# wenz116/lang2seg

Hardware: AMD Instinct MI355X
Metric: train images/sec (cycle loss on), 600×1000 input, at 1/2/4/8 MI355X (higher is better)
Workload: dtype bf16; 1 GPU; train_cycle.sh step: ResNet-101 C4 + 7 spatial dynamic filters + att2in2 cycle loss, 600x1000 image, 20-token expression (V=3349), 12000->2000 proposals, 256 RoIs, per-GPU batch 1; variant=cycle, parallelism=dp1

## Files before the change

### include/lang2seg_hip.h

```cpp
#ifndef LANG2SEG_HIP_H
#define LANG2SEG_HIP_H
#include <stdint.h>
#ifdef __HIPCC__
#include <hip/hip_runtime.h>
#else
typedef struct ihipStream_t* hipStream_t;
#endif
#ifdef __cplusplus
extern "C" {
#endif

#define L2S_F32 0
#define L2S_BF16 1

int l2s_version(void);

#define L2S_CONV_RELU 1
#define L2S_CONV_OUT_F32 4
#define L2S_CONV_DECONV2X2 8
#define L2S_CONV_SCATTER 16
#define L2S_ALGO_AUTO 0
#define L2S_ALGO_STAGED 1
#define L2S_ALGO_DMA 2
#define L2S_ALGO_DMA_STAMPED 4
// ... 274 lines not shown
int l2s_prep_geometry(int h, int w, int target_size, int max_size, double* scale, int* oh, int* ow);
int l2s_prep_image(const uint8_t* img_bgr, int h, int w, double mean_b, double mean_g, double mean_r, double scale,
                   int oh, int ow, float* out, hipStream_t s);
long l2s_rle_ws_words(int total_counts, int oh, int ow);
int l2s_rle_to_mask(const uint32_t* cnts, const int* offs, int n, int total_counts, int h, int w, int oh, int ow,
                    uint32_t* ws, uint8_t* out, hipStream_t s);

typedef struct { int roi; int cls; float box[4]; int hit; int reserved; long long I; long long U; } l2s_eval_record;
int l2s_eval_pick(const float* cls_prob, const float* bbox_pred, const float* rois, const int* nkeep, int post, int ncls, float im_scale,
                  int im_h, int im_w, const float* gt_box, int bbox_reg, l2s_eval_record* rec, float* mask_roi, int* mask_label, hipStream_t s);
int l2s_eval_mask_iou(const float* mask_prob, int ms, l2s_eval_record* rec, const uint8_t* gt, int Hs, int Ws, int ih, int iw,
                      uint8_t* canvas, hipStream_t s);

int l2s_stream_fork(hipStream_t from, hipStream_t to);
int l2s_event_record(int slot, hipStream_t s);
int l2s_event_wait(int slot, hipStream_t s);
int l2s_memset_async(void* p, int value, size_t bytes, hipStream_t s);
int l2s_memcpy_d2d_async(void* dst, const void* src, size_t bytes, hipStream_t s);
void* l2s_tape_begin(const hipStream_t* streams, int n);
int l2s_tape_end(void* tape);
long l2s_tape_size(void* tape);
int l2s_tape_run(void* tape, const hipStream_t* streams, int n);
int l2s_tape_pause(int on);
int l2s_tape_mark(void);
int l2s_tape_time_event(hipStream_t s);
int l2s_time_event_elapsed(int a, int b, float* ms);
int l2s_tape_segments(void* tape);
int l2s_tape_run_segment(void* tape, const hipStream_t* streams, int n, int seg);
int l2s_tape_destroy(void* tape);

typedef struct { long offset; long count; int row_len; int weight_decay; long rowscale_off; float lr_mult;
                 int chunk0;
                 int flags;
                 int reserved; } l2s_sgd_seg;
int l2s_sgd_momentum_range(float* param, float* grad, float* mom, const l2s_sgd_seg* segs, int nseg, const float* rowscale,
                           float lr, float momentum, float wd, float grad_scale, void* shadow, int shadow_dtype, int flags,
                           long lo, long hi, int chunk_lo, int chunk_hi, hipStream_t s);
int l2s_sgd_momentum_range_g16(float* param, const void* grad_bf16, long grad_lo, float* mom, const l2s_sgd_seg* segs, int nseg, const float* rowscale,
                               float lr, float momentum, float wd, float grad_scale, void* shadow, int shadow_dtype,
                               long lo, long hi, int chunk_lo, int chunk_hi, hipStream_t s);
int l2s_sgd_chunk(void);
int l2s_sgd_momentum(float* param, float* grad, float* mom, const l2s_sgd_seg* segs, int nseg, const float* rowscale,
                     float lr, float momentum, float wd, float grad_scale, void* shadow ,
                     int shadow_dtype, int clear_grad ,
                     hipStream_t s);

#ifdef __cplusplus
}
#endif
#endif
```

### lang2seg_amd/_lib.py

```python
import ctypes as C
import os

_HERE = os.path.dirname(os.path.abspath(__file__))
LIB_PATH = os.path.join(_HERE, 'lib', 'liblang2seg_hip.so')
F32, BF16 = 0, 1

vp, i32, i64, f32, u64, sz = C.c_void_p, C.c_int, C.c_long, C.c_float, C.c_uint64, C.c_size_t


class ConvDesc(C.Structure):
    _fields_ = [('x', vp), ('w', vp), ('y', vp), ('bias', vp), ('add', vp), ('ref', vp),
                ('n_img', i32), ('IH', i32), ('IW', i32), ('Cin', i32), ('OH', i32), ('OW', i32), ('Cout', i32),
                ('KH', i32), ('KW', i32), ('stride', i32), ('pad', i32),
                ('ldx', i32), ('ldy', i32), ('ldadd', i32), ('ldref', i32), ('flags', i32),
                ('out_h', i32), ('out_w', i32), ('out_stride', i32), ('tile', i32), ('split_k', i32), ('xcd_mode', i32), ('algo', i32), ('ws', vp), ('ws_floats', sz), ('prio', i32)]


class RoiBlock0Desc(C.Structure):
    _fields_ = [('feat', vp), ('rois', vp), ('w1', vp), ('b1', vp), ('w2', vp), ('b2', vp), ('pooled', vp), ('y1', vp), ('y2', vp),
                ('H', i32), ('W', i32), ('C', i32), ('R', i32), ('P', i32), ('N1', i32), ('N2', i32), ('spatial_scale', C.c_float), ('debug', i32)]


class WgradDesc(C.Structure):
    _fields_ = [('dy', vp), ('x', vp), ('dw', vp),
# ... 7 lines not shown
                ('lddy', i32 * 2), ('ldx', i32 * 2), ('dw', vp),
                ('nseg', i32), ('Cin', i32), ('Cout', i32), ('KH', i32), ('KW', i32), ('stride', i32), ('pad', i32),
                ('split', i32), ('ws_off', i64), ('flags', i32), ('reserved', i32)]


class TransposeDesc(C.Structure):
    _fields_ = [('src', vp), ('scale', vp), ('dst', vp), ('Cout', i32), ('taps', i32), ('Cin', i32), ('force_f32', i32)]


class LstmFwdDir(C.Structure):
    _fields_ = [(n, C.c_void_p) for n in ('w_hh', 'b_hh', 'gates_in', 'h_prev', 'c_prev', 'c', 'h', 'act', 'gates_out')]


class LstmBwdDir(C.Structure):
    _fields_ = [(n, C.c_void_p) for n in ('w_hh_T', 'dgates_next', 'dh_ext', 'dc_in', 'act', 'c_prev', 'c', 'dgates', 'dc_prev')]


class Bottleneck64Desc(C.Structure):
    _fields_ = [(n, vp) for n in ('a', 'x', 'w2', 'w3', 'wd', 'w1n', 'b2', 'b3', 'bd', 'b1n', 'y', 'a_next')] + [(n, i32) for n in ('H', 'W', 'Cx')]


class CapRecurFwdArgs(C.Structure):
    _fields_ = [(n, vp) for n in ('w_h2h', 'b_h2h', 'w_h2att', 'b_h2att', 'patt', 'aw', 'ab', 'P', 'b_a2c', 'sums', 'hs', 'cs', 'save', 'tanh_ws', 'wgt', 'state')] + \
               [(n, i32) for n in ('S', 'R', 'AH', 'L')]


class CapRecurBwdArgs(C.Structure):
    _fields_ = [(n, vp) for n in ('w_h2h', 'w_h2att', 'P', 'aw', 'save', 'cs', 'wgt', 'tanh_ws', 'dho', 'dsums', 'da2c', 'ddot', 'datt_h', 'state')] + \
               [(n, i32) for n in ('S', 'R', 'AH', 'L', 'ld_ddot', 'ld_datt_h')]


class SgdSeg(C.Structure):
    _fields_ = [('offset', i64), ('count', i64), ('row_len', i32), ('weight_decay', i32), ('rowscale_off', i64),
                ('lr_mult', f32), ('chunk0', i32), ('flags', i32), ('reserved', i32)]


CONV_RELU, CONV_OUT_F32, CONV_DECONV2X2, CONV_SCATTER = 1, 4, 8, 16
LOSS_RPN_CLS, LOSS_RPN_BOX, LOSS_CLS, LOSS_BOX, LOSS_MASK, LOSS_CAP, LOSS_TOTAL, LOSS_RESPONSE = range(8)

SIGS = {
    'l2s_version': (i32, []),
    'l2s_conv_plan_name': (C.c_char_p, [vp, i32]),
    'l2s_roialign_block0_fwd': (i32, [C.POINTER(RoiBlock0Desc), vp]),
    'l2s_conv_igemm': (i32, [C.POINTER(ConvDesc), i32, vp]),
    'l2s_conv_wgrad': (i32, [C.POINTER(WgradDesc), i32, vp]),
    'l2s_wgrad_ws_bytes': (sz, [C.POINTER(WgradDesc), i32]),
    'l2s_wgrad_variant': (i32, [i32, i32, i32, i32, i32, i32, i32, i64, i32]),
    'l2s_wgrad_tiles': (i64, [i32, i32, i32, i32, i32]),
    'l2s_conv_wgrad_grouped': (i32, [vp, vp, i32, i32, i32, vp, sz, vp]),
    'l2s_weight_cast': (i32, [vp, vp, vp, i32, i32, i32, i32, vp]),
    'l2s_weight_transpose': (i32, [vp, vp, vp, i32, i32, i32, i32, vp]),
    'l2s_colsum': (i32, [vp, i32, i32, i32, vp, vp, i64, i32, vp]),
    'l2s_weight_transpose_batched': (i32, [vp, i32, i32, i32, vp]),
    'l2s_stem_conv': (i32, [vp, vp, vp, vp, vp, i32, i32, i32, i32, i32, vp]),
    'l2s_stem_pack_bytes': (C.c_size_t, []),
    'l2s_stem_pack': (i32, [vp, vp, vp]),
    'l2s_stem_pool_bf16': (i32, [vp, vp, vp, vp, vp, i32, i32, i32, i32, i32, i32, vp]),
    'l2s_maxpool3x3s2': (i32, [vp, vp, i32, i32, i32, i32, i32, i32, vp]),
    'l2s_fill_f32': (i32, [vp, f32, i64, vp]),
    'l2s_cast': (i32, [vp, i32, vp, i32, i64, vp]),
    'l2s_add3': (i32, [vp, vp, vp, vp, i64, i32, vp]),
    'l2s_avgpool_fwd': (i32, [vp, vp, i32, i32, i32, i32, vp]),
    'l2s_avgpool_bwd': (i32, [vp, vp, vp, vp, i32, i32, i32, i32, vp]),
    'l2s_adaptive_pool_fwd': (i32, [vp, vp, vp, i32, i32, i32, i32, i32, i32, i32, vp]),
    'l2s_adaptive_pool_bwd': (i32, [vp, i32, i32, i32, vp, vp, vp, i32, i32, i32, i32, i32, i32, vp]),
    'l2s_mask_downsample': (i32, [vp, vp, i32, i32, i32, i32, vp]),
    'l2s_dropout_mask': (i32, [vp, i64, f32, vp, u64, vp]),
# ... 150 lines not shown
```

### lang2seg_amd/csrc/misc_kernels.hip

```cpp
#include "common.h"
#include "../../include/lang2seg_hip.h"

namespace {

__device__ __forceinline__ uint64_t mix64(uint64_t z) {
  z += 0x9E3779B97F4A7C15ull;
  z = (z ^ (z >> 30)) * 0xBF58476D1CE4E5B9ull;
  z = (z ^ (z >> 27)) * 0x94D049BB133111EBull;
  return z ^ (z >> 31);
}

inline int grid_for(long n, int block = 256, int cap = 2048) {
  long g = (n + block - 1) / block;
  if (g < 1) g = 1;
  return (int)(g > cap ? cap : g);
}

__global__ void weight_cast_kernel(const float* __restrict__ src, const float* __restrict__ scale, void* dst,
                                   long per_row, long total, int dt) {
  for (long i = blockIdx.x * (long)blockDim.x + threadIdx.x; i < total; i += (long)gridDim.x * blockDim.x) {
    float v = src[i];
    if (scale) v *= scale[i / per_row];
    stx(dst, i, dt, v);
  }
// ... 465 lines not shown
  const int bw = x1 - x0, n = (y1 - y0) * bw;
  float s = 0.f;
  for (int i = lane; i < n; i += 64) { int yy = y0 + i / bw, xx = x0 + i % bw; s += (float)mask[(long)yy * W + xx]; }
  s = wave_sum(s);
  if (lane == 0) out[o] = (s / (float)n >= 0.5f) ? 1.f : 0.f;
}

__global__ void counter_inc_kernel(uint64_t* c) { *c += 1; }
__global__ void stamp_kernel(uint64_t* out) { *out = wall_clock64(); }
__global__ void dropout_kernel(float* m, long n, float p, const uint64_t* seed_dev, uint64_t salt) {
  const uint64_t seed = mix64(*seed_dev * 0x9E3779B97F4A7C15ull + salt);
  const float keep = 1.f - p, inv = keep > 0.f ? 1.f / keep : 0.f;
  for (long i = blockIdx.x * (long)blockDim.x + threadIdx.x; i < n; i += (long)gridDim.x * blockDim.x) {
    uint32_t r = (uint32_t)(mix64(seed * 0x100000001B3ull + (uint64_t)i) >> 40);
    m[i] = ((float)r * (1.f / 16777216.f) < keep) ? inv : 0.f;
  }
}
__global__ void keys_kernel(uint32_t* k, long n, const uint64_t* seed_dev, uint64_t salt) {
  const uint64_t seed = mix64(*seed_dev * 0x9E3779B97F4A7C15ull + salt);
  for (long i = blockIdx.x * (long)blockDim.x + threadIdx.x; i < n; i += (long)gridDim.x * blockDim.x)
    k[i] = (uint32_t)(mix64(seed * 0x100000001B3ull + (uint64_t)i) >> 32);
}

constexpr int SGD_CHUNK = 4096;
__device__ __forceinline__ void sgd_elem(float g, float& w, float& m, float rs, float gscale, float lwd, float momentum, float llr) {
  const float gg = g * gscale * rs + lwd * w;
  m = momentum * m + gg;
  w = w - llr * m;
}
__global__ __launch_bounds__(256) void sgd_kernel(float* __restrict__ param, float* __restrict__ grad, float* __restrict__ mom,
                                                  const l2s_sgd_seg* __restrict__ segs, int nseg, const float* __restrict__ rowscale,
                                                  float lr, float momentum, float wd, float gscale, void* shadow, int sdt, int flags,
                                                  long lo, long hi, int chunk_lo, int chunk_hi, const bf16_t* __restrict__ g16, long g16_lo) {
  const bool clear = flags & 1, shadow_only = flags & 2;
  const int c0 = segs[0].chunk0;
  int total = segs[nseg - 1].chunk0 - c0 + (int)((segs[nseg - 1].count + SGD_CHUNK - 1) / SGD_CHUNK);
  if (chunk_hi >= 0 && chunk_hi < total) total = chunk_hi;
  for (int c = (chunk_lo > 0 ? chunk_lo : 0) + blockIdx.x; c < total; c += gridDim.x) {
    int slo = 0, shi = nseg - 1;
    while (slo < shi) {
      const int mid = (slo + shi + 1) >> 1;
      if (segs[mid].chunk0 - c0 <= c) slo = mid; else shi = mid - 1;
    }
    const l2s_sgd_seg sg = segs[slo];
    const long base = (long)(c - (sg.chunk0 - c0)) * SGD_CHUNK;
    const int n = (int)((sg.count - base) < SGD_CHUNK ? (sg.count - base) : SGD_CHUNK);
    const float lwd = sg.weight_decay ? wd : 0.f;
    const float llr = lr * sg.lr_mult;
    const bool clr = clear && !(sg.flags & 1);
    const long o0 = sg.offset + base;
    const bool inside = o0 >= lo && o0 + n <= hi;
    const bool vec = inside && ((sg.offset & 3) == 0) && (sg.rowscale_off < 0 || (sg.row_len & 3) == 0);
    const int nv = vec ? (n >> 2) : 0;
    float4 g4[4], w4[4], m4[4];
#pragma unroll
    for (int j = 0; j < 4; ++j) {
      const int v = threadIdx.x + j * 256;
      if (v < nv) {
        w4[j] = *(const float4*)(param + o0 + 4 * v);
        if (!shadow_only) {
          if (g16) {
            const uint2 pk = *(const uint2*)(g16 + (o0 + 4 * v - g16_lo));
            g4[j] = make_float4(bf2f((bf16_t)(pk.x & 0xffffu)), bf2f((bf16_t)(pk.x >> 16)), bf2f((bf16_t)(pk.y & 0xffffu)), bf2f((bf16_t)(pk.y >> 16)));
          } else g4[j] = *(const float4*)(grad + o0 + 4 * v);
          m4[j] = *(const float4*)(mom + o0 + 4 * v);
        }
      }
    }
#pragma unroll
    for (int j = 0; j < 4; ++j) {
      const int v = threadIdx.x + j * 256;
      if (v >= nv) continue;
      const long o = o0 + 4 * v;
      const float rs = sg.rowscale_off >= 0 ? rowscale[sg.rowscale_off + (unsigned)(base + 4 * v) / (unsigned)sg.row_len] : 1.f;
      float ww[4] = {w4[j].x, w4[j].y, w4[j].z, w4[j].w};
      if (!shadow_only) {
        float gg[4] = {g4[j].x, g4[j].y, g4[j].z, g4[j].w}, mm[4] = {m4[j].x, m4[j].y, m4[j].z, m4[j].w};
#pragma unroll
        for (int e = 0; e < 4; ++e) sgd_elem(gg[e], ww[e], mm[e], rs, gscale, lwd, momentum, llr);
        *(float4*)(mom + o) = make_float4(mm[0], mm[1], mm[2], mm[3]);
        *(float4*)(param + o) = make_float4(ww[0], ww[1], ww[2], ww[3]);
        if (clr && !g16) *(float4*)(grad + o) = make_float4(0.f, 0.f, 0.f, 0.f);
// ... 220 lines not shown
```

### lang2seg_amd/nets/network.py

```python
import numpy as np
import os
import torch

from .. import ops as O
from .._lib import F32, BF16, LOSS_CAP
from ..model.config import cfg
from .params import ParamStore
from . import anchors as ANC


class ConvOp(object):

    def __init__(self, net, wkey, Cin, Cout, k=1, stride=1, pad=0, bias_key=None, need_dgrad=True, group=None, Cout_pad=None, full_map=False):
        self.net, self.wkey, self.Cin, self.Cout, self.k, self.stride, self.pad = net, wkey, Cin, Cout, k, stride, pad
        self.full_map = bool(full_map and k > 1 and pad == 0 and stride == 1)
        self.t_taps, self.t_cin = (1, k * k * Cin) if self.full_map else (k * k, Cin)
        self.bias_key, self.need_dgrad, self.group = bias_key, need_dgrad, group
        self.Np = Cout if Cout_pad is None else Cout_pad
        self.prio = 1 if str(wkey).startswith(('resnet.layer1.', 'resnet.layer2.', 'resnet.layer3.')) and getattr(net, 'chain_prio', True) else 0
        P = net.P
        taps = k * k
        cnt = self.Np * taps * Cin
        if group is not None:
            self.trainable = True
# ... 500 lines not shown
        raise NotImplementedError

    def train(self, mode=True):
        self.training = mode
        return self

    def eval(self):
        return self.train(False)

    def cuda(self):
        return self

    def state_dict(self):
        self.join_update()
        dp = getattr(self, 'dp', None)
        if dp is not None and getattr(dp, 'master_stale', False):
            raise RuntimeError('state_dict() of a sharded data-parallel run: call net.dp.gather_master() on every rank first')
        return self.P.state_dict()

    def load_state_dict(self, sd, strict=False):
        self.join_update()
        self.P.load_state_dict(sd, strict)
        self.refresh_weights(full=True)

    def named_parameters(self):
        from .params import from_internal
        self.join_update()
        dp = getattr(self, 'dp', None)
        if dp is not None and getattr(dp, 'master_stale', False):
            raise RuntimeError('named_parameters() of a sharded data-parallel run: call net.dp.gather_master() on every rank first')
        for k in self.P.trainable:
            yield k, from_internal(k, self.P.view(k), self.P.shapes[k])

    def refresh_weights(self, full=False):
        if full:
            for c in self.convs:
                if not c.trainable:
                    O.weight_cast(c.w_master, c.scale, c.wf, c.Np, c.k * c.k, c.Cin)
        if getattr(self, '_tr_table', None) is None:
            from .._lib import TransposeDesc
            items = [c for c in self.convs if c.wb is not None] + list(getattr(self, 'extra_transposes', []))
            arr = (TransposeDesc * len(items))()
            for i, c in enumerate(items):
                arr[i].src, arr[i].scale, arr[i].dst = c.w_master.data_ptr(), (c.scale.data_ptr() if c.scale is not None else None), c.wb.data_ptr()
                arr[i].Cout, arr[i].taps, arr[i].Cin, arr[i].force_f32 = c.Np, getattr(c, 't_taps', c.k * c.k), getattr(c, 't_cin', c.Cin), int(getattr(c, 'force_f32', 0))
                if self.dt == BF16 and isinstance(c, ConvOp) and c.trainable and not arr[i].force_f32:
                    arr[i].src, arr[i].scale, arr[i].force_f32 = c.wf.data_ptr(), None, 2
            self._tr_table = torch.frombuffer(bytearray(bytes(arr)), dtype=torch.uint8).to(self.device)
            self._tr_n = len(items)
            self._tr_tiles = sum(((c.Cin + 63) // 64) * ((c.Np + 63) // 64) * c.k * c.k for c in items)
        if self.use_streams and not full:
            S = self.streams()
            self.sfork(torch.cuda.current_stream(), S['tr'])
            with torch.cuda.stream(S['tr']):
                O.weight_transpose_batched(self._tr_table, self._tr_n, self._tr_tiles, self.dt)
            self._tr_pending = True
        else:
            O.weight_transpose_batched(self._tr_table, self._tr_n, self._tr_tiles, self.dt)

    update_on_wg = False
    defer_heads = False
    conv_algo = None
    roi_pdma = False
    layer1_fused = True
    cap_persistent = True
    _precleared = frozenset()
    prio_floor = 0
    cap_map_prio = 0
    rpn_wgrad_early = False
    rpn_bwd_early = True
    join_before_layer1 = False
    stem_mfma = True
    wgrad_overwrite = True
    update_clears_grad = False
    SLOT_UPDATE_REST = 0
    SLOT_UPDATE_L2 = 1
    SLOT_WGRADS = 2
    update_split = False
    layer2_side = False

    def join_update(self, full=True, layer2_only=False):
        if self.use_streams and self.update_on_wg:
            if layer2_only and self.update_split and not self.defer_heads and not getattr(self, '_pass_without_step', False):
                O.event_wait(self.SLOT_UPDATE_L2, torch.cuda.current_stream())
                if not self.layer2_side:
                    O.event_wait(self.SLOT_WGRADS, torch.cuda.current_stream())
            elif self.defer_heads and not full:
                O.event_wait(self.SLOT_UPDATE_REST, torch.cuda.current_stream())
            else:
                self.sfork(self.streams()['wg'], torch.cuda.current_stream())
                if self.layer2_side:
# ... 37 lines not shown
                r = cache['_sent_ref_host'][idx]
                gm = cache['_gt_masks_ref'][r:r + 1]
            else:
                gm = torch.from_numpy(np.ascontiguousarray(blobs['gt_masks'][idx:idx + 1], dtype=np.uint8)).to(dev)
            cache[key] = dict(
                gt_boxes=torch.from_numpy(np.ascontiguousarray(blobs['gt_boxes'][idx:idx + 1], dtype=np.float32)).to(dev),
                gt_masks=gm,
                labels=torch.from_numpy(lab[0]).to(dev), T=max_len, S=S,
                cap_in=torch.from_numpy(cap[0, :S].copy()).to(dev), cap_tgt=torch.from_numpy(cap[0, 1:S + 1].copy()).to(dev),
                cap_mask=torch.from_numpy(cm[0, 1:S + 1].copy()).to(dev))
        d = dict(cache[key])
        d['data'] = cache['data']
        d['im_info'] = np.asarray(blobs['im_info'], dtype=np.float32).reshape(-1)[:3]
        return d

    def train_step(self, blobs, idx, train_op):
        loss = self.train_step_async(blobs, idx, train_op)
        vals = loss.cpu().numpy()
        if not np.isfinite(vals[np.asarray(self._loss_slots())]).all():
            self.check_cap_recur()
        return tuple(float(vals[i]) for i in self._loss_slots())

    def check_cap_recur(self):
        from .._lib import L2SError
        st = getattr(self, '_cap_state', None)
        if st is None:
            return
        torch.cuda.synchronize()
        err = [int(s[1].item()) for s in st]
        if any(err):
            for s in st:
                s.zero_()
            raise L2SError('captioner recurrence: a workgroup of the resident %s launch gave up waiting for its peers (not co-resident); the '
                           'exchange state was reset - set Network.cap_persistent = False to run the per-token launches' %
                           ' / '.join(n for n, e in zip(('forward', 'backward'), err) if e))

    def _loss_slots(self):
        from .variants import loss_names, SLOT
        return [SLOT[k] for k in loss_names(getattr(self, 'variant', 'cycle'))]

    def _loss_names(self):
        from .variants import loss_names
        return loss_names(getattr(self, 'variant', 'cycle'))

    def train_step_async(self, blobs, idx, train_op):
        dev = self.upload_blob(blobs, idx)
        self._early_op = train_op if (self.dp is None and self.use_streams and self.parity is None
                                      and getattr(train_op, 'early', False) and str(self.device).startswith('cuda')) else None
        if getattr(self, 'use_tape', False) and self.use_streams and self.parity is None:
            loss = self.tape_step(dev, train_op)
        elif getattr(self, 'use_graph', False) and self.dp is None and self.parity is None:
            loss = self.graph_step(dev, train_op)
        else:
            loss = self.forward_backward(dev)
            if self.dp is not None:
                self.dp.finish()
            train_op.step()
        self._early_op = None
        self._step += 1
        return loss

    def train_step_with_summary(self, blobs, idx, train_op):
        r = self.train_step(blobs, idx, train_op)
        return r + ([(n, v) for n, v in zip(self._loss_names(), r)],)

    def get_summary(self, blobs, idx):
        was = self.training
# ... 6 lines not shown
```

### lang2seg_amd/nets/params.py

```python
import ctypes as C
import numpy as np
import torch

from .. import ops as O
from .._lib import SgdSeg

RESNET_LAYERS = {50: [3, 4, 6, 3], 101: [3, 4, 23, 3], 152: [3, 8, 36, 3]}
BN_EPS = 1e-5


def to_internal(name, t):
    if name == 'vgg.classifier.0.weight':
        return t.view(t.shape[0], 512, 7, 7).permute(0, 2, 3, 1).contiguous().view(t.shape[0], -1)
    if t.dim() == 4 and name == 'mask_up_sampling.weight':
        return t.permute(0, 2, 3, 1).contiguous()
    if t.dim() == 4:
        return t.permute(0, 2, 3, 1).contiguous()
    return t.contiguous()


def from_internal(name, t, ref_shape):
    if name == 'vgg.classifier.0.weight':
        return t.view(ref_shape[0], 7, 7, 512).permute(0, 3, 1, 2).contiguous().view(ref_shape)
    if len(ref_shape) == 4 and name == 'mask_up_sampling.weight':
# ... 292 lines not shown
            g, b = self.frozen[bn + '.weight'], self.frozen[bn + '.bias']
            m, v = self.frozen[bn + '.running_mean'], self.frozen[bn + '.running_var']
            s = g / torch.sqrt(v + BN_EPS)
            self.bn_scale[k].copy_(s)
            self.bn_bias[k].copy_(b - m * s)
            if k in self.rowscale_off:
                o = self.rowscale_off[k]
                self.rowscale[o:o + s.numel()].copy_(s)

    def param_group(self, k, double_bias=False, bias_decay=False, lang_lr_mult=None, from_frcn=False, gamma=0.1):
        from .variants import SOLVERS, LANG_LR_KEYS
        mult = SOLVERS[self.variant]['lang_lr_mult'] if lang_lr_mult is None else float(lang_lr_mult)
        is_bias = 'bias' in k
        if from_frcn:
            f = 1.0 if 'mask' in k else float(gamma)
        else:
            f = mult if any(t in k for t in LANG_LR_KEYS) else 1.0
        if is_bias and double_bias:
            f *= 2.0
        return f, (1 if (not is_bias or bias_decay) else 0)

    def build_segments(self, double_bias=False, bias_decay=False, lang_lr_mult=None, from_frcn=False, gamma=0.1):
        segs = []
        for k in self.trainable:
            cnt = int(np.prod(self.shapes[k]))
            sg = SgdSeg()
            sg.offset, sg.count = self.offsets[k], cnt
            sg.row_len = cnt // self.shapes[k][0] if k in self.rowscale_off else 1
            sg.lr_mult, sg.weight_decay = self.param_group(k, double_bias, bias_decay, lang_lr_mult, from_frcn, gamma)
            sg.rowscale_off = self.rowscale_off.get(k, -1)
            segs.append(sg)
        self.seg_rule = (bool(double_bias), bool(bias_decay), lang_lr_mult, bool(from_frcn), float(gamma))
        CH = int(O.sgd_chunk())

        def table(seq):
            run = 0
            for g in seq:
                g.chunk0 = run
                run += -(-int(g.count) // CH)
            arr = (SgdSeg * len(seq))(*seq)
            self._seg_tables.append(arr)
            return torch.frombuffer(bytearray(bytes(arr)), dtype=torch.uint8).to(self.device)
        self._seg_tables, self._ow_key = [], frozenset()
        self.nseg = len(segs)
        self.seg_ends = [int(g.offset + g.count) for g in segs]
        self.seg_offs = [int(g.offset) for g in segs]
        self.seg_chunks = [-(-int(g.count) // CH) for g in segs]
        self.seg_chunk0 = [sum(self.seg_chunks[:i]) for i in range(len(segs))]
        self.sgd_chunk = CH
        self.seg_size = C.sizeof(SgdSeg)
        self.segs_dev = table(segs)
        lo, hi = self.defer_range
        cp = lambda g: SgdSeg.from_buffer_copy(bytes(g))
        rest = [cp(g) for g in segs if not (lo <= g.offset < hi)]
        late = [cp(g) for g in segs if lo <= g.offset < hi]
        self.n_rest = len(rest)
        self.segs_split_dev = table(rest + late)
        return self.nseg

    def mark_overwritten(self, ptrs):
        key = frozenset(ptrs)
        if key == self._ow_key:
            return
        base = self.grad.data_ptr()
        torch.cuda.synchronize() if self.grad.is_cuda else None
        for arr, dev in zip(self._seg_tables, (self.segs_dev, self.segs_split_dev)):
            for g in arr:
                was, now = g.flags & 1, int(base + 4 * int(g.offset) in key)
                if was and not now:
                    self.grad[int(g.offset):int(g.offset + g.count)].zero_()
                g.flags = now
            dev.copy_(torch.frombuffer(bytearray(bytes(arr)), dtype=torch.uint8))
        torch.cuda.synchronize() if self.grad.is_cuda else None
        self._ow_key = key

    def stale_marked(self, s0, s1, fresh):
        if not self._ow_key:
            return []
        base = self.grad.data_ptr()
        return [base + 4 * o for o in self.seg_offs[s0:s1] if (base + 4 * o) in self._ow_key and (base + 4 * o) not in fresh]

    def chunk_range(self, lo, hi):
        import bisect
        s0 = bisect.bisect_right(self.seg_ends, lo)
        s1 = bisect.bisect_left(self.seg_offs, hi)
        if s0 >= s1:
            return 0, 0
        c_lo = self.seg_chunk0[s0] + max(0, lo - self.seg_offs[s0]) // self.sgd_chunk
        last = s1 - 1
        c_hi = self.seg_chunk0[last] + min(self.seg_chunks[last], -(-(min(hi, self.seg_ends[last]) - self.seg_offs[last]) // self.sgd_chunk))
        return c_lo, c_hi

    def refresh_shadow_full(self):
        if not hasattr(self, 'segs_dev'):
            self.build_segments()
        zero = torch.zeros_like(self.grad)
        O.sgd_momentum(self.param, zero, self.mom, self.segs_dev, self.nseg, self.rowscale, 0.0, 1.0, 0.0, 0.0, shadow=self.shadow)
```

### lang2seg_amd/nets/resnet_v1.py

```python
import os
import numpy as np
import torch

from .. import ops as O
from .._lib import F32, BF16
from ..model.config import cfg
from .network import Network, ConvOp, Bottleneck
from .params import ParamStore
from .variants import solver_cfg
from . import anchors as ANC

f32 = torch.float32


class resnetv1(Network):
    variant = 'cycle'

    def __init__(self, opt, batch_size=1, num_layers=50, variant=None):
        Network.__init__(self, batch_size=batch_size)
        from .variants import VARIANTS
        if variant is not None:
            self.variant = variant
        self.var = VARIANTS[self.variant]
        self._num_layers = num_layers
# ... 76 lines not shown
        class _T(object):
            pass
        P = self.P
        self.wT, self.extra_transposes = {}, []
        def add(name, src, N, K, dst=None, f32=1):
            e = _T(); e.w_master, e.scale, e.Np, e.k, e.Cin, e.force_f32 = src, None, N, 1, K, f32
            e.wb = torch.zeros(K * N, dtype=torch.float32, device=self.device) if dst is None else dst
            self.extra_transposes.append(e)
            if dst is None:
                self.wT[name] = (e.wb, N, K)
        for sfx in ['', '_reverse']:
            w = 'rnn_encoder.rnn.weight_hh_l0'
            add(w + sfx, P.view(w + sfx), *P.shapes[w + sfx])
        capk = ['caption_model.core.h2h.weight', 'caption_model.core.attention.h2att.weight']
        if not (self.cap_projected and self.opt['rnn_size'] <= 1024):
            capk.append('caption_model.core.a2c.weight')
        for k in (capk if self.var['cap'] is not None else []):
            add(k, P.view(k), *P.shapes[k])
        add('mask_up', P.view('mask_up_sampling.weight'), 2048, 4 * 256, dst=self.up_wT, f32=0)

    def bwd_x(self, dy, name, dx, M, accumulate=False, lddy=None, mul=None):
        if M == 1 and name in self.wT:
            assert mul is None
            wT, N, K = self.wT[name]
            O.linear_fwd(dy, wT, None, dx, M, K, N, accumulate=accumulate, ldx=N if lddy is None else lddy, ldw=N)
            return
        P = self.P
        w = P.view(name)
        N, K = P.shapes[name]
        nws = O.linear_bwd_x_ws_floats(M, N, K)
        ws = self.buf('bwdx.ws.' + name, (nws,), f32) if nws else None
        O.linear_bwd_x(dy, w, dx, M, N, K, accumulate=accumulate, lddy=lddy, mul=mul, ws=ws)

    def refresh_weights(self, full=False):
        if not hasattr(self, 'extra_transposes'):
            self._make_transposes()
        if full and getattr(self, '_stem_pack', None) is not None:
            w1 = self.P.frozen['resnet.conv1.weight']
            self._stem_pack, self._stem_pack_ver = O.stem_pack(w1, self._stem_pack), (w1.data_ptr(), w1._version)
        Network.refresh_weights(self, full)

    def _drop(self, name, shape, p):
        if not self.training or p <= 0.0:
            return None
        if self.parity is not None:
            m = (self.parity.get('drops') or {}).get(name)
            return m
        m = self.buf('drop.' + name, shape, f32)
        O.dropout_mask(m, p, self.seed_counter(), 1000003 * sum(map(ord, name)) + getattr(self, 'rank_seed', 0))
        return m

    def _keys(self, name, n):
        if self.parity is not None and self.parity.get(name) is not None:
            return self.parity[name]
        k = self.buf('keys.' + name, (n,), torch.int32)
        O.random_keys(k, self.seed_counter(), 7777 + 1000003 * sum(map(ord, name)) + getattr(self, 'rank_seed', 0))
        return k

    def _encoder_fwd(self, d):
        P, T = self.P, d['T']
        Hh, E = self.opt['rnn_hidden_size'], self.opt['word_embedding_size']
        t = self.t
        emb = self.buf('enc.emb', (T, E), f32)
        t['enc.drop'] = self._drop('word', (T, E), self.opt['word_drop_out'])
        O.embed_fwd(P.view('rnn_encoder.embedding.weight'), d['labels'], t['enc.drop'], emb, T, E, False)
        x = self.buf('enc.x', (T, Hh), f32)
        O.linear_fwd(emb, P.view('rnn_encoder.mlp.0.weight'), P.view('rnn_encoder.mlp.0.bias'), x, T, Hh, E, act=1)
        hidden = self.buf('enc.hidden', (2 * Hh,), f32)
        st = []
        for di, sfx in enumerate(['', '_reverse']):
            g = self.buf('enc.gates' + sfx, (T, 4 * Hh), f32)
            O.linear_fwd(x, P.view('rnn_encoder.rnn.weight_ih_l0' + sfx), P.view('rnn_encoder.rnn.bias_ih_l0' + sfx), g, T, 4 * Hh, Hh)
            st.append(dict(g=g, hs=self.buf('enc.hfull' + sfx, (T + 1, Hh), f32), cs=self.buf('enc.cfull' + sfx, (T + 1, Hh), f32),
# ... 829 lines not shown
```

### lang2seg_amd/optim.py

```python
import bisect

import torch

from . import ops as O


class SGD(object):
    def __init__(self, net, lr, momentum=0.9, weight_decay=1e-4, grad_scale=1.0, keep_grad=False):
        self.net = net
        self.lr, self.momentum, self.weight_decay, self.grad_scale = float(lr), float(momentum), float(weight_decay), float(grad_scale)
        self.param_groups = [self.__dict__]
        self.side_active = bool(self.side and getattr(net, 'use_streams', False) and hasattr(net, 'flush_wgrads'))
        if self.side_active:
            net.update_on_wg = True
        self._early = bool(type(self)._early and not self.defer)
        self.defer_active = bool(self.defer and self.side_active and not self._early and hasattr(net, 'wgq') and getattr(net, 'dp', None) is None)
        net.defer_heads = self.defer_active
        net.update_split = bool(self.side_active and getattr(net, 'dp', None) is None and not self.defer_active)
        net.layer2_side = bool(net.update_split and self.layer2_side and getattr(net.P, 'fixed_blocks', 1) == 1 and not getattr(net.P, 'is_vgg', False))
        dp = getattr(net, 'dp', None)
        if dp is not None and getattr(dp, 'shard_update', None) is True:
            dp.shard_update = self
        if dp is not None and getattr(dp, 'bucket_update', None) is True:
            dp.bucket_update = self
# ... 39 lines not shown
            P.mark_overwritten(P._ow_key - frozenset(stale))
        S = net.streams()
        tr = S['tr']
        net.sfork(torch.cuda.current_stream(), tr)
        for name in ('wg', 'wg2', 'lang', 'cap'):
            net.sfork(S[name], tr)
        with torch.cuda.stream(tr):
            self._launch(self._seg_done, hi)
            net._mark('partial update %s (tr)' % stage)
        self._seg_done = hi

    side = True

    layer2_side = True
    defer = False

    def _mark_overwritten(self):
        net = self.net
        if self.clear_grad and not self.defer_active and getattr(net, 'wgrad_overwrite', False):
            net.P.mark_overwritten(getattr(net, '_fresh', ()))

    def step(self):
        P = self.net.P
        net = self.net
        net._bwd_pending = 0
        net._pass_without_step = False
        if getattr(getattr(net, 'dp', None), 'shard_update', None) is not None:
            gathered = bool(getattr(net.dp, 'gather_shadow', False))
            if self.side_active and net.use_streams:
                net.flush_wgrads('final')
                with torch.cuda.stream(net.streams()['wg']):
                    if not gathered:
                        self.refresh_shadow()
                    net.refresh_weights()
                    net._mark('update done (wg)')
                return
            if hasattr(net, 'join_wgrad'):
                net.join_wgrad()
            if not gathered:
                self.refresh_shadow()
            net.refresh_weights()
            return
        if getattr(getattr(net, 'dp', None), 'bucket_update', None) is self:
            if self.side_active and net.use_streams:
                net.flush_wgrads('final')
                self._mark_overwritten()
                with torch.cuda.stream(net.streams()['wg']):
                    net.refresh_weights()
                    net._mark('update done (wg)')
                return
            if hasattr(net, 'join_wgrad'):
                net.join_wgrad()
            self._mark_overwritten()
            net.refresh_weights()
            return
        if self.side_active and net.use_streams:
            net.flush_wgrads('final')
            self._mark_overwritten()
            S = net.streams()
            early_tail = bool(self._seg_done and net.update_split and not self.defer_active and getattr(net.wgq, 'V5_STREAM', 'wg') != 'tr')
            side2 = bool(early_tail and getattr(net, '_layer2_on_side', False))
            net._layer2_on_side = False
            if not side2:
                net.sfork(S['wg2'], S['wg'])
            if getattr(net.wgq, 'V5_STREAM', 'wg') == 'tr':
                net.sfork(S['tr'], S['wg'])
            O.event_record(net.SLOT_WGRADS, S['wg'])
            if early_tail:
                T = S['wg2'] if side2 else S['wg']
                net.sfork(torch.cuda.current_stream(), T)
                with torch.cuda.stream(T):
                    self._launch(self._seg_done, P.nseg)
                    O.event_record(net.SLOT_UPDATE_L2, T)
                    net._mark('update of layer2 done')
                for k in ('wg2', 'lang', 'cap', 'tr'):
                    net.sfork(S[k], S['wg'])
                net.sfork(torch.cuda.current_stream(), S['wg'])
                with torch.cuda.stream(S['wg']):
                    net.refresh_weights()
                    net._mark('update done (wg)')
                self._seg_done = 0
                return
            for k in ('wg2', 'lang', 'cap'):
                net.sfork(S[k], S['wg'])
            if self._seg_done or getattr(net.wgq, 'V5_STREAM', 'wg') == 'tr':
                net.sfork(S['tr'], S['wg'])
            net.sfork(torch.cuda.current_stream(), S['wg'])
# ... 55 lines not shown
```

Baseline: 227.0 img/s.

## Fuse conv weight transpose into SGD update via tiled shadow writes

The SGD kernel gains a tiled mode for conv weight segments. It processes 64x64 (cout, cin) tiles per tap and writes the updated weights both to the shadow copy and, through a shared-memory transpose, to the transposed/flipped weight buffer the backward convs use. Segments covered this way are dropped from the separate batched weight-transpose launch, which saves a full read of the master weights and one kernel pass per step. The cost is extra shared memory and syncthreads in the SGD kernel, plus more complex range and chunk handling for partial updates. Paths where the shadow is gathered or bucketed fall back to the full transpose.

```diff
diff --git a/include/lang2seg_hip.h b/include/lang2seg_hip.h
--- a/include/lang2seg_hip.h
+++ b/include/lang2seg_hip.h
@@ -330,7 +330,8 @@
 typedef struct { long offset; long count; int row_len; int weight_decay; long rowscale_off; float lr_mult;
                  int chunk0;
                  int flags;
-                 int reserved; } l2s_sgd_seg;
+                 int tiled;
+                 void* tdst; int t_cout, t_taps, t_cin; int t_pad; } l2s_sgd_seg;
 int l2s_sgd_momentum_range(float* param, float* grad, float* mom, const l2s_sgd_seg* segs, int nseg, const float* rowscale,
                            float lr, float momentum, float wd, float grad_scale, void* shadow, int shadow_dtype, int flags,
                            long lo, long hi, int chunk_lo, int chunk_hi, hipStream_t s);
diff --git a/lang2seg_amd/_lib.py b/lang2seg_amd/_lib.py
--- a/lang2seg_amd/_lib.py
+++ b/lang2seg_amd/_lib.py
@@ -63,7 +63,8 @@
 
 class SgdSeg(C.Structure):
     _fields_ = [('offset', i64), ('count', i64), ('row_len', i32), ('weight_decay', i32), ('rowscale_off', i64),
-                ('lr_mult', f32), ('chunk0', i32), ('flags', i32), ('reserved', i32)]
+                ('lr_mult', f32), ('chunk0', i32), ('flags', i32), ('tiled', i32),
+                ('tdst', vp), ('t_cout', i32), ('t_taps', i32), ('t_cin', i32), ('t_pad', i32)]
 
 
 CONV_RELU, CONV_OUT_F32, CONV_DECONV2X2, CONV_SCATTER = 1, 4, 8, 16
diff --git a/lang2seg_amd/csrc/misc_kernels.hip b/lang2seg_amd/csrc/misc_kernels.hip
--- a/lang2seg_amd/csrc/misc_kernels.hip
+++ b/lang2seg_amd/csrc/misc_kernels.hip
@@ -521,6 +521,7 @@
                                                   const l2s_sgd_seg* __restrict__ segs, int nseg, const float* __restrict__ rowscale,
                                                   float lr, float momentum, float wd, float gscale, void* shadow, int sdt, int flags,
                                                   long lo, long hi, int chunk_lo, int chunk_hi, const bf16_t* __restrict__ g16, long g16_lo) {
+  __shared__ float tile[64][65];
   const bool clear = flags & 1, shadow_only = flags & 2;
   const int c0 = segs[0].chunk0;
   int total = segs[nseg - 1].chunk0 - c0 + (int)((segs[nseg - 1].count + SGD_CHUNK - 1) / SGD_CHUNK);
@@ -537,6 +538,95 @@
     const float lwd = sg.weight_decay ? wd : 0.f;
     const float llr = lr * sg.lr_mult;
     const bool clr = clear && !(sg.flags & 1);
+    if (sg.tiled) {
+      const int t = c - (sg.chunk0 - c0), tci = sg.t_cin >> 6;
+      const int q = t / tci, tap = q % sg.t_taps, otap = sg.t_taps - 1 - tap;
+      const int co0 = (q / sg.t_taps) << 6, ci0 = (t - q * tci) << 6;
+      const long rstride = (long)sg.t_taps * sg.t_cin;
+      const long e0 = ((long)co0 * sg.t_taps + tap) * sg.t_cin + ci0;
+      const long first = sg.offset + e0, last = first + 63 * rstride + 64;
+      if (last <= lo || first >= hi) continue;
+      if (first >= lo && last <= hi) {
+        float4 g4[4], w4[4], m4[4];
+#pragma unroll
+        for (int j = 0; j < 4; ++j) {
+          const int v = threadIdx.x + j * 256;
+          const long o = first + (v >> 4) * rstride + ((v & 15) << 2);
+          w4[j] = *(const float4*)(param + o);
+          if (!shadow_only) {
+            if (g16) {
+              const uint2 pk = *(const uint2*)(g16 + (o - g16_lo));
+              g4[j] = make_float4(bf2f((bf16_t)(pk.x & 0xffffu)), bf2f((bf16_t)(pk.x >> 16)), bf2f((bf16_t)(pk.y & 0xffffu)), bf2f((bf16_t)(pk.y >> 16)));
+            } else g4[j] = *(const float4*)(grad + o);
+            m4[j] = *(const float4*)(mom + o);
+          }
+        }
+        if (shadow) __syncthreads();
+#pragma unroll
+        for (int j = 0; j < 4; ++j) {
+          const int v = threadIdx.x + j * 256, r = v >> 4, c4 = (v & 15) << 2;
+          const long o = first + r * rstride + c4;
+          const float rs = sg.rowscale_off >= 0 ? rowscale[sg.rowscale_off + (unsigned)(e0 + r * rstride + c4) / (unsigned)sg.row_len] : 1.f;
+          float ww[4] = {w4[j].x, w4[j].y, w4[j].z, w4[j].w};
+          if (!shadow_only) {
+            float gg[4] = {g4[j].x, g4[j].y, g4[j].z, g4[j].w}, mm[4] = {m4[j].x, m4[j].y, m4[j].z, m4[j].w};
+#pragma unroll
+            for (int e = 0; e < 4; ++e) sgd_elem(gg[e], ww[e], mm[e], rs, gscale, lwd, momentum, llr);
+            *(float4*)(mom + o) = make_float4(mm[0], mm[1], mm[2], mm[3]);
+            *(float4*)(param + o) = make_float4(ww[0], ww[1], ww[2], ww[3]);
+            if (clr && !g16) *(float4*)(grad + o) = make_float4(0.f, 0.f, 0.f, 0.f);
+          }
+          if (shadow) {
+#pragma unroll
+            for (int e = 0; e < 4; ++e) { ww[e] *= rs; tile[r][c4 + e] = ww[e]; }
+            if (sdt) {
+              uint2 pk; pk.x = (uint32_t)f2bf(ww[0]) | ((uint32_t)f2bf(ww[1]) << 16); pk.y = (uint32_t)f2bf(ww[2]) | ((uint32_t)f2bf(ww[3]) << 16);
+              *(uint2*)((bf16_t*)shadow + o) = pk;
+            } else *(float4*)((float*)shadow + o) = make_float4(ww[0], ww[1], ww[2], ww[3]);
+          }
+        }
+        if (shadow) {
+          __syncthreads();
+          const int cg = (threadIdx.x & 7) << 3;
+#pragma unroll
+          for (int pass = 0; pass < 2; ++pass) {
+            const int r = (threadIdx.x >> 3) + pass * 32;
+            float v[8];
+#pragma unroll
+            for (int e = 0; e < 8; ++e) v[e] = tile[cg + e][r];
+            const long o = ((long)(ci0 + r) * sg.t_taps + otap) * sg.t_cout + co0 + cg;
+            if (sdt) {
+              uint4 pk;
+              pk.x = (uint32_t)f2bf(v[0]) | ((uint32_t)f2bf(v[1]) << 16); pk.y = (uint32_t)f2bf(v[2]) | ((uint32_t)f2bf(v[3]) << 16);
+              pk.z = (uint32_t)f2bf(v[4]) | ((uint32_t)f2bf(v[5]) << 16); pk.w = (uint32_t)f2bf(v[6]) | ((uint32_t)f2bf(v[7]) << 16);
+              *(uint4*)((bf16_t*)sg.tdst + o) = pk;
+            } else {
+              *(float4*)((float*)sg.tdst + o) = make_float4(v[0], v[1], v[2], v[3]);
+              *(float4*)((float*)sg.tdst + o + 4) = make_float4(v[4], v[5], v[6], v[7]);
+            }
+          }
+        }
+      } else {
+        for (int i = threadIdx.x; i < SGD_CHUNK; i += 256) {
+          const int r = i >> 6, cc = i & 63;
+          const long e = e0 + r * rstride + cc, o = sg.offset + e;
+          if (o < lo || o >= hi) continue;
+          const float rs = sg.rowscale_off >= 0 ? rowscale[sg.rowscale_off + (unsigned)e / (unsigned)sg.row_len] : 1.f;
+          float w = param[o];
+          if (!shadow_only) {
+            float m = mom[o];
+            sgd_elem(g16 ? bf2f(g16[o - g16_lo]) : grad[o], w, m, rs, gscale, lwd, momentum, llr);
+            mom[o] = m; param[o] = w;
+            if (clr && !g16) grad[o] = 0.f;
+          }
+          if (shadow) {
+            stx(shadow, o, sdt, w * rs);
+            stx(sg.tdst, ((long)(ci0 + cc) * sg.t_taps + otap) * sg.t_cout + co0 + r, sdt, w * rs);
+          }
+        }
+      }
+      continue;
+    }
     const long o0 = sg.offset + base;
     const bool inside = o0 >= lo && o0 + n <= hi;
     const bool vec = inside && ((sg.offset & 3) == 0) && (sg.rowscale_off < 0 || (sg.row_len & 3) == 0);
diff --git a/lang2seg_amd/nets/network.py b/lang2seg_amd/nets/network.py
--- a/lang2seg_amd/nets/network.py
+++ b/lang2seg_amd/nets/network.py
@@ -556,31 +556,47 @@
         for k in self.P.trainable:
             yield k, from_internal(k, self.P.view(k), self.P.shapes[k])
 
-    def refresh_weights(self, full=False):
+    def refresh_weights(self, full=False, covered=True):
         if full:
             for c in self.convs:
                 if not c.trainable:
                     O.weight_cast(c.w_master, c.scale, c.wf, c.Np, c.k * c.k, c.Cin)
-        if getattr(self, '_tr_table', None) is None:
+        first = getattr(self, '_tr_table', None) is None
+        if first:
             from .._lib import TransposeDesc
             items = [c for c in self.convs if c.wb is not None] + list(getattr(self, 'extra_transposes', []))
             arr = (TransposeDesc * len(items))()
+            P = self.P
+            p0, want = P.param.data_ptr(), {}
             for i, c in enumerate(items):
                 arr[i].src, arr[i].scale, arr[i].dst = c.w_master.data_ptr(), (c.scale.data_ptr() if c.scale is not None else None), c.wb.data_ptr()
                 arr[i].Cout, arr[i].taps, arr[i].Cin, arr[i].force_f32 = c.Np, getattr(c, 't_taps', c.k * c.k), getattr(c, 't_cin', c.Cin), int(getattr(c, 'force_f32', 0))
+                off = (c.w_master.data_ptr() - p0) // 4
+                if not arr[i].force_f32 and 0 <= off < P.total and O.dt_of(P.shadow) == self.dt and O.dt_of(c.wb) == self.dt:
+                    want[off] = (c.wb.data_ptr(), arr[i].Cout, arr[i].taps, arr[i].Cin, i)
                 if self.dt == BF16 and isinstance(c, ConvOp) and c.trainable and not arr[i].force_f32:
                     arr[i].src, arr[i].scale, arr[i].force_f32 = c.wf.data_ptr(), None, 2
+            tiles = lambda d: ((d.Cin + 63) // 64) * ((d.Cout + 63) // 64) * d.taps
             self._tr_table = torch.frombuffer(bytearray(bytes(arr)), dtype=torch.uint8).to(self.device)
-            self._tr_n = len(items)
-            self._tr_tiles = sum(((c.Cin + 63) // 64) * ((c.Np + 63) // 64) * c.k * c.k for c in items)
+            self._tr_n, self._tr_items = len(items), items
+            self._tr_tiles = sum(tiles(d) for d in arr)
+            taken = P.set_transposed({o: e[:4] for o, e in want.items()}) if self.device != 'cpu' else set()
+            skip = set(e[4] for o, e in want.items() if o in taken)
+            rest = [arr[i] for i in range(len(items)) if i not in skip]
+            self._tr_rest_n, self._tr_rest_tiles = len(rest), sum(tiles(d) for d in rest)
+            self._tr_rest = torch.frombuffer(bytearray(bytes((TransposeDesc * max(len(rest), 1))(*rest))), dtype=torch.uint8).to(self.device)
+        if full or first or not covered:
+            tab = (self._tr_table, self._tr_n, self._tr_tiles)
+        else:
+            tab = (self._tr_rest, self._tr_rest_n, self._tr_rest_tiles)
         if self.use_streams and not full:
             S = self.streams()
             self.sfork(torch.cuda.current_stream(), S['tr'])
             with torch.cuda.stream(S['tr']):
-                O.weight_transpose_batched(self._tr_table, self._tr_n, self._tr_tiles, self.dt)
+                O.weight_transpose_batched(tab[0], tab[1], tab[2], self.dt)
             self._tr_pending = True
         else:
-            O.weight_transpose_batched(self._tr_table, self._tr_n, self._tr_tiles, self.dt)
+            O.weight_transpose_batched(tab[0], tab[1], tab[2], self.dt)
 
     update_on_wg = False
     defer_heads = False
@@ -684,7 +700,8 @@
             for s in st:
                 s.zero_()
             raise L2SError('captioner recurrence: a workgroup of the resident %s launch gave up waiting for its peers (not co-resident); the '
-                           'exchange state was reset - set Network.cap_persistent = False to run the per-token launches' %
+                           'exchange state was reset, but the step\'s NaN has already gone through the update: weights and momentum are '
+                           'poisoned - restart from the last snapshot, with Network.cap_persistent = False to run the per-token launches' %
                            ' / '.join(n for n, e in zip(('forward', 'backward'), err) if e))
 
     def _loss_slots(self):
diff --git a/lang2seg_amd/nets/params.py b/lang2seg_amd/nets/params.py
--- a/lang2seg_amd/nets/params.py
+++ b/lang2seg_amd/nets/params.py
@@ -348,6 +348,8 @@
             segs.append(sg)
         self.seg_rule = (bool(double_bias), bool(bias_decay), lang_lr_mult, bool(from_frcn), float(gamma))
         CH = int(O.sgd_chunk())
+        for g in segs:
+            self._tile_seg(g, CH)
 
         def table(seq):
             run = 0
@@ -363,6 +365,7 @@
         self.seg_offs = [int(g.offset) for g in segs]
         self.seg_chunks = [-(-int(g.count) // CH) for g in segs]
         self.seg_chunk0 = [sum(self.seg_chunks[:i]) for i in range(len(segs))]
+        self.seg_tiled = [bool(g.tiled) for g in segs]
         self.sgd_chunk = CH
         self.seg_size = C.sizeof(SgdSeg)
         self.segs_dev = table(segs)
@@ -373,6 +376,41 @@
         self.n_rest = len(rest)
         self.segs_split_dev = table(rest + late)
         return self.nseg
+
+    tr_map = None
+
+    def _tile_seg(self, g, CH):
+        g.tiled, g.tdst, g.t_cout, g.t_taps, g.t_cin = 0, None, 0, 0, 0
+        e = (self.tr_map or {}).get(int(g.offset))
+        if e is None:
+            return False
+        dst, cout, taps, cin = e
+        ok = (cout * taps * cin == int(g.count) and cout % 64 == 0 and cin % 64 == 0 and CH == 4096 and g.offset % 4 == 0 and dst % 16 == 0
+              and (g.rowscale_off < 0 or g.row_len % 4 == 0))
+        if ok:
+            g.tiled, g.tdst, g.t_cout, g.t_taps, g.t_cin = 1, dst, cout, taps, cin
+        return ok
+
+    def set_transposed(self, entries):
+        self.tr_map = dict(entries)
+        if not hasattr(self, 'segs_dev'):
+            self.build_segments()
+        torch.cuda.synchronize() if self.grad.is_cuda else None
+        taken = set()
+        for arr, dev in zip(self._seg_tables, (self.segs_dev, self.segs_split_dev)):
+            for g in arr:
+                if self._tile_seg(g, self.sgd_chunk):
+                    taken.add(int(g.offset))
+            dev.copy_(torch.frombuffer(bytearray(bytes(arr)), dtype=torch.uint8))
+        torch.cuda.synchronize() if self.grad.is_cuda else None
+        self.seg_tiled = [bool(g.tiled) for g in self._seg_tables[0]]
+        return taken
+
+    def segs_flat_dev(self):
+        arr = (SgdSeg * self.nseg).from_buffer_copy(bytes(self._seg_tables[0]))
+        for g in arr:
+            g.tiled, g.tdst = 0, None
+        return torch.frombuffer(bytearray(bytes(arr)), dtype=torch.uint8).to(self.device)
 
     def mark_overwritten(self, ptrs):
         key = frozenset(ptrs)
@@ -402,9 +440,10 @@
         s1 = bisect.bisect_left(self.seg_offs, hi)
         if s0 >= s1:
             return 0, 0
-        c_lo = self.seg_chunk0[s0] + max(0, lo - self.seg_offs[s0]) // self.sgd_chunk
+        c_lo = self.seg_chunk0[s0] + (0 if self.seg_tiled[s0] else max(0, lo - self.seg_offs[s0]) // self.sgd_chunk)
         last = s1 - 1
-        c_hi = self.seg_chunk0[last] + min(self.seg_chunks[last], -(-(min(hi, self.seg_ends[last]) - self.seg_offs[last]) // self.sgd_chunk))
+        c_hi = self.seg_chunk0[last] + (self.seg_chunks[last] if self.seg_tiled[last] else
+                                        min(self.seg_chunks[last], -(-(min(hi, self.seg_ends[last]) - self.seg_offs[last]) // self.sgd_chunk)))
         return c_lo, c_hi
 
     def refresh_shadow_full(self):
diff --git a/lang2seg_amd/nets/resnet_v1.py b/lang2seg_amd/nets/resnet_v1.py
--- a/lang2seg_amd/nets/resnet_v1.py
+++ b/lang2seg_amd/nets/resnet_v1.py
@@ -132,13 +132,13 @@
         ws = self.buf('bwdx.ws.' + name, (nws,), f32) if nws else None
         O.linear_bwd_x(dy, w, dx, M, N, K, accumulate=accumulate, lddy=lddy, mul=mul, ws=ws)
 
-    def refresh_weights(self, full=False):
+    def refresh_weights(self, full=False, covered=True):
         if not hasattr(self, 'extra_transposes'):
             self._make_transposes()
         if full and getattr(self, '_stem_pack', None) is not None:
             w1 = self.P.frozen['resnet.conv1.weight']
             self._stem_pack, self._stem_pack_ver = O.stem_pack(w1, self._stem_pack), (w1.data_ptr(), w1._version)
-        Network.refresh_weights(self, full)
+        Network.refresh_weights(self, full, covered)
 
     def _drop(self, name, shape, p):
         if not self.training or p <= 0.0:
diff --git a/lang2seg_amd/optim.py b/lang2seg_amd/optim.py
--- a/lang2seg_amd/optim.py
+++ b/lang2seg_amd/optim.py
@@ -95,27 +95,27 @@
                 with torch.cuda.stream(net.streams()['wg']):
                     if not gathered:
                         self.refresh_shadow()
-                    net.refresh_weights()
+                    net.refresh_weights(covered=not gathered)
                     net._mark('update done (wg)')
                 return
             if hasattr(net, 'join_wgrad'):
                 net.join_wgrad()
             if not gathered:
                 self.refresh_shadow()
-            net.refresh_weights()
+            net.refresh_weights(covered=not gathered)
             return
         if getattr(getattr(net, 'dp', None), 'bucket_update', None) is self:
             if self.side_active and net.use_streams:
                 net.flush_wgrads('final')
                 self._mark_overwritten()
                 with torch.cuda.stream(net.streams()['wg']):
-                    net.refresh_weights()
+                    net.refresh_weights(covered=False)
                     net._mark('update done (wg)')
                 return
             if hasattr(net, 'join_wgrad'):
                 net.join_wgrad()
             self._mark_overwritten()
-            net.refresh_weights()
+            net.refresh_weights(covered=False)
             return
         if self.side_active and net.use_streams:
             net.flush_wgrads('final')
```

Result: slower. 224.5 img/s (-1.1%).
